# JuliaMeshless/WhatsThePoint.jl

Hardware: AMD Instinct MI355X
Metric: Mpoints/sec per repel iter (k=21 KNN+force) (higher is better)
Workload: dtype f32

## Files before the change

### include/wtp.h

```cpp
#ifndef WTP_H
#define WTP_H

#include <stdint.h>

#ifdef __cplusplus
extern "C" {
#endif

typedef struct wtp_ctx wtp_ctx;

typedef enum wtp_status {
    WTP_OK = 0,
    WTP_ERR_ARG = 1,
    WTP_ERR_OOM = 2,
    WTP_ERR_HIP = 3,
    WTP_ERR_STATE = 4,
    WTP_ERR_NO_DEVICE = 5
} wtp_status;

typedef enum wtp_dtype { WTP_F32 = 0, WTP_F64 = 1 } wtp_dtype;

typedef enum wtp_force_kind {
    WTP_FORCE_INVERSE_DISTANCE = 0,
    WTP_FORCE_SPACING_EQUILIBRIUM = 1,
// ... 165 lines not shown
                   int64_t n_owned, const wtp_spacing_desc* spacing, const wtp_force_desc* force, int k,
                   double alpha_lo, double alpha_max);
int wtp_block_step(wtp_ctx* ctx, wtp_step_stats* stats, wtp_block_info* info);
int wtp_block_run(wtp_ctx* ctx, int n_iters, double* conv_out, wtp_step_stats* last, wtp_block_info* info);
int wtp_block_run_until(wtp_ctx* ctx, int max_iters, double tol, int stall_after, double cv_target, double* conv_out,
                        int* n_done, int* reason, wtp_step_stats* last);
int wtp_block_get(wtp_ctx* ctx, void* d_xyz_out, int64_t* d_gid_out, int64_t cap, int64_t* n_owned);
int wtp_block_close(wtp_ctx* ctx);
int wtp_block_grid(int nranks, int p_out[3]);
int wtp_block_morton_rank(int ix, int iy, int iz, const int p[3]);
int wtp_comm_exchange_peers(wtp_ctx* ctx, int n_msgs, const int* peers, const void* const* d_send, const int64_t* n_send,
                            void* const* d_recv, const int64_t* n_recv);
int wtp_comm_allgather_dev(wtp_ctx* ctx, const void* d_send, void* d_recv, int64_t bytes);

int wtp_relax_set_coverage(wtp_ctx* ctx, int axis, double lo, double hi);
int wtp_relax_set_coverage_box(wtp_ctx* ctx, const double lo[3], const double hi[3]);

int wtp_relax_set_fixed_dev(wtp_ctx* ctx, const void* d_fixed4, int64_t n_fixed_new);


int wtp_timers_get(wtp_ctx* ctx, double out[4]);
int wtp_timers_reset(wtp_ctx* ctx);
int wtp_debug_diag(wtp_ctx* ctx, unsigned long long out[16]);

int wtp_gen_uniform_dev(wtp_ctx* ctx, uint64_t seed, int64_t first, int64_t n, int dim, int dtype,
                        void* d_out);

#ifdef __cplusplus
}
#endif
#endif
```

### whatsthepoint.jl_amd/_lib.py

```python
from __future__ import annotations

import ctypes as C
import os
import subprocess

_HERE = os.path.dirname(os.path.abspath(__file__))
CSRC = os.path.join(_HERE, "csrc")
SO_PATH = os.environ.get("WTP_LIB") or os.path.join(CSRC, "libwtp.so")

WTP_OK, WTP_ERR_ARG, WTP_ERR_OOM, WTP_ERR_HIP, WTP_ERR_STATE, WTP_ERR_NO_DEVICE = range(6)
WTP_F32, WTP_F64 = 0, 1
WTP_SPACING_CONSTANT, WTP_SPACING_PER_POINT, WTP_SPACING_LOGLIKE, WTP_SPACING_BOUNDARY_LAYER = range(4)


class WtpError(RuntimeError):

    def __init__(self, code, msg):
        super().__init__(f"libwtp status {code}: {msg}")
        self.code = code


class WtpArgumentError(ValueError):
    """WTP_ERR_ARG: the reference throws ArgumentError for the same input (src/repel.jl:74)."""

# ... 85 lines not shown
                                    C.POINTER(C.c_double), C.POINTER(C.c_double), C.POINTER(_vp), C.POINTER(_vp), _i64,
                                    C.POINTER(_i64)]),
    "wtp_relax_set_coverage": (_i, [_vp, _i, _d, _d]),
    "wtp_relax_set_coverage_box": (_i, [_vp, C.POINTER(C.c_double), C.POINTER(C.c_double)]),
    "wtp_comm_unique_id": (_i, [_vp, _vp]),
    "wtp_comm_init": (_i, [_vp, _vp, _i, _i]),
    "wtp_comm_finalize": (_i, [_vp]),
    "wtp_comm_exchange_rows": (_i, [_vp, _i, _i, _vp, _i64, _vp, _i64, _vp, _vp, _i64, C.POINTER(_i64), C.POINTER(_i64)]),
    "wtp_comm_allreduce_stats": (_i, [_vp, C.POINTER(StepStats)]),
    "wtp_block_set_transport": (_i, [_vp, C.POINTER(Transport)]),
    "wtp_block_open": (_i, [_vp, C.POINTER(BlockDesc), _vp, _vp, _i64, C.POINTER(SpacingDesc), C.POINTER(ForceDesc), _i, _d, _d]),
    "wtp_block_step": (_i, [_vp, C.POINTER(StepStats), C.POINTER(BlockInfo)]),
    "wtp_block_run": (_i, [_vp, _i, _vp, C.POINTER(StepStats), C.POINTER(BlockInfo)]),
    "wtp_block_run_until": (_i, [_vp, _i, _d, _i, _d, _vp, C.POINTER(_i), C.POINTER(_i), C.POINTER(StepStats)]),
    "wtp_block_get": (_i, [_vp, _vp, _vp, _i64, C.POINTER(_i64)]),
    "wtp_block_close": (_i, [_vp]),
    "wtp_block_grid": (_i, [_i, C.POINTER(_i)]),
    "wtp_block_morton_rank": (_i, [_i, _i, _i, C.POINTER(_i)]),
    "wtp_comm_exchange_peers": (_i, [_vp, _i, C.POINTER(_i), C.POINTER(_vp), C.POINTER(_i64), C.POINTER(_vp), C.POINTER(_i64)]),
    "wtp_comm_allgather_dev": (_i, [_vp, _vp, _vp, _i64]),
    "wtp_timers_get": (_i, [_vp, C.POINTER(_d)]),
    "wtp_timers_reset": (_i, [_vp]),
    "wtp_debug_diag": (_i, [_vp, C.POINTER(C.c_ulonglong)]),
    "wtp_gen_uniform_dev": (_i, [_vp, C.c_uint64, _i64, _i64, _i, _i, _vp]),
}

_lib = None


def build(verbose: bool = False) -> str:
    res = subprocess.run(["make", "-C", CSRC, "-j4"], capture_output=True, text=True)
    if res.returncode != 0:
        raise RuntimeError("building libwtp.so failed:\n" + res.stdout[-4000:] + res.stderr[-4000:])
    if verbose:
        print(res.stdout[-2000:])
    return SO_PATH


def load():
    global _lib
    if _lib is not None:
        return _lib
    if not os.path.exists(SO_PATH):
        raise ImportError(
            f"{SO_PATH} is missing: build it with `python -c 'import __graft_entry__ as g; g.build()'` "
            "(hipcc --offload-arch=gfx950).  There is no CPU fallback."
# ... 23 lines not shown
```

### whatsthepoint.jl_amd/csrc/wtp_api.hip

```cpp
#include <cmath>
#include <cstdlib>
#include <cstring>
#include <type_traits>

#include "wtp_internal.hpp"

namespace wtp {

static thread_local std::string g_create_err;

int fail(wtp_ctx* ctx, int code, const std::string& msg) {
    if (ctx)
        ctx->err = msg;
    else
        g_create_err = msg;
    return code;
}

int ensure(wtp_ctx* ctx, DevBuf& b, size_t bytes) {
    if (bytes == 0) bytes = 16;
    if (b.cap >= bytes) return WTP_OK;
    if (b.p) {
        hipFree(b.p);
        b.p = nullptr;
// ... 1070 lines not shown

static int relax_f64_ksel_sweep(wtp_ctx* ctx, SearchArgs<double>& a, int* sp) {
    RelaxState& r = ctx->relax;
    const int64_t n = r.n;
    const int kc = 24;
    int rc;
    if ((rc = ensure(ctx, ctx->f64k_s64, sizeof(double4) * (size_t)n))) return rc;
    if ((rc = ensure(ctx, ctx->f64k_slot, sizeof(int32_t) * (size_t)n))) return rc;
    if ((rc = ensure(ctx, ctx->f64k_lists, sizeof(int32_t) * 2 * (size_t)n))) return rc;
    if ((rc = ensure(ctx, ctx->f64k_cnt, 64))) return rc;
    const double4* snap = (const double4*)a.snap;
    SearchArgs<float> b{};
    b.fb_list = (int32_t*)ctx->f64k_lists.p;
    b.fb_count = (int32_t*)ctx->f64k_cnt.p;
    b.fb2_list = (int32_t*)ctx->f64k_lists.p + n;
    b.fb2_count = (int32_t*)ctx->f64k_cnt.p + 4;
    b.stop = ctx->stop_dev;
    b.diag = a.diag;
    *sp = span_begin(ctx, 0);
    WTP_HIP(ctx, hipMemsetAsync(ctx->f64k_cnt.p, 0, 64, ctx->stream));
    b.counters_cleared = 1;
    std::swap(ctx->grid, ctx->grid_b);
    std::swap(ctx->cell_start, ctx->cell_start_b);
    const void* ncells_session = ctx->ncells_dev;
    const bool box_session = ctx->box_active;
    const double* org4 = nullptr;
    rc = f64_candidates(ctx, snap, n, 3, kc, r.f64k_tune, b, *sp, &org4, [&](float4* sorted32) {
        return launch_relabel_slots(ctx, snap, sorted32, (double4*)ctx->f64k_s64.p, (int32_t*)ctx->f64k_slot.p, n);
    });
    std::swap(ctx->grid, ctx->grid_b);
    std::swap(ctx->cell_start, ctx->cell_start_b);
    ctx->ncells_dev = ncells_session;
    ctx->box_active = box_session;
    if (rc) return rc;
    return launch_refine_sweep_f64(ctx, a, (const double4*)ctx->f64k_s64.p, (const int32_t*)ctx->f64k_slot.p,
                                   (const int32_t*)ctx->cand_idx.p, (const float*)ctx->cand_dist.p, org4);
}

static bool grid_reusable(const wtp_ctx* ctx, int64_t n_fixed_next, bool head_swapped) {
    const RelaxState& r = ctx->relax;
    const bool head_ok = !head_swapped || (r.shard_grid_reuse && r.grid_fixed > 0 &&
                                           std::llabs((long long)(n_fixed_next - r.grid_fixed)) * 10 <= (long long)r.grid_fixed + 640);
    return r.grid_age < kGridReuseMax && !r.moved_by_hand && head_ok && !ctx->box_active;
}

static bool head_remeasures(const RelaxState& r, int64_t n_fixed_new) {
    const int64_t n_new = r.n - r.n_fixed + n_fixed_new;
    return r.cs2_bx > 0 && std::llabs((long long)(n_fixed_new - r.tuned_fixed)) * 20 > (long long)n_new;
}

template <typename T> static SweepRoute sweep_route(const wtp_ctx* ctx, const RelaxState& r) {
    if (ctx->force_generic) return SweepRoute::Exact;
    const bool clipped = r.force.kind == WTP_FORCE_CLIPPED_SPACING;
    if (clipped && r.k >= 2 && r.k < 32 && !ctx->full_select && !r.cs_disabled) {
// ... 132 lines not shown
            if (r.route == SweepRoute::Cs2) {
                Grid<float> hgf;
                memcpy(&hgf, &hg, sizeof(hgf));
                if ((rc = cs2_tune(ctx, r, hgf, rho_eff))) return rc;
            } else if (route_cs(r.route)) {
                int hc = (int)(HCELLS * rho_eff * 1.15) + 128;
                hc = (hc + 63) / 64 * 64;
                r.brick_hcap = hc < 640 ? 640 : (hc > 2560 ? 2560 : hc);
            }
            if (r.route == SweepRoute::Ksel) {
                if ((rc = ksel_tune<T>(ctx, r.tune, in, out, r.n, r.dim, r.k, hg, rho_eff))) return rc;
                g.rho = r.tune.rho;
            }
            r.tune.valid = true;
            r.tuned_fixed = r.n_fixed;
            r.grid_fixed = r.n_fixed;
            r.grid_age = 0;
        } else {
            const bool reuse = grid_reusable(ctx, r.n_fixed, ctx->hash_view.active);
            ctx->reuse_grid = reuse;
            r.grid_age = reuse ? r.grid_age + 1 : 0;
            if (!reuse) r.grid_fixed = r.n_fixed;
            ctx->topology_build = r.route == SweepRoute::F64Ksel;
            rc = build_hash<T>(ctx, in, out, r.n, r.dim, r.k, 0.0, g.rho, g.min_cell, r.tune.scale);
            ctx->topology_build = false;
            ctx->reuse_grid = false;
        }
        r.last_rho_cs = g.rho;
        span_end(ctx, sp);
        ctx->hash_view.active = false;
        if (rc) return rc;
        r.pending.active = false;
        r.bufS = t;
        r.bufP = t;
        r.have_tree = true;
        r.sweeps_since_rebuild = 0;
        r.moved_by_hand = false;
    }
    if (spacing_on_device(r.spacing_kind)) {
        int sps = span_begin(ctx, 2);
        rc = launch_spacing_session<T>(ctx, (const Pt<T>*)ctx->pts[r.bufP].p, r.n, r.n_fixed, ctx->kd_nodes.p, ctx->kd_m,
                                       r.spacing_kind, r.sp_p0, r.sp_p1, r.sp_p2, (T*)ctx->spacing_pp.p,
                                       (int32_t*)ctx->sp_hint.p - r.aux_off, r.have_tree ? (const int32_t*)ctx->cell_start.p : nullptr,
                                       ctx->grid.p, (Pt<T>*)ctx->sp_cert.p - r.aux_off);
        span_end(ctx, sps);
        if (rc) return rc;
    }
    const bool fresh = (r.bufS == r.bufP);
    const int o = pick_free(r, r.bufS, r.bufP);
    if ((rc = ensure(ctx, ctx->pts[o], sizeof(Pt<T>) * (size_t)(r.n + r.shard_extra)))) return rc;
// ... 31 lines not shown
        }
    }
    if ((rc = ensure(ctx, ctx->diag, 128))) return rc;
    a.diag = (unsigned long long*)ctx->diag.p;
    a.brick_hcap = route_cs(r.route) ? r.brick_hcap : (r.route == SweepRoute::Ksel ? r.tune.hcap : 0);
    a.cs2_bx = route_cs(r.route) ? r.cs2_bx : 0;
    a.cs2_chunked = (r.spacing_kind != WTP_SPACING_CONSTANT || r.cs2_rho > 1.6) ? 1 : 0;
    a.ksel_bx = r.route == SweepRoute::Ksel ? r.tune.bx : 0;
    if (r.route == SweepRoute::Ksel) a.cap_count = (float)ksel_cap_count(r.k);
    if (route == SweepRoute::Select || route == SweepRoute::Cs || route == SweepRoute::Cs2) {
        a.gamma_cap = (T)kGammaCapSweep;
        a.cap_count = (float)(4.18879 * kGammaCapSweep * kGammaCapSweep * kGammaCapSweep * ctx->rho * (a.k + 1) / 22.0);
    }
    if (route == SweepRoute::Cs64 || route == SweepRoute::Cs64Wave) a.gamma_cap = (T)kGammaCap;
    a.tnn_frac = (T)kTnnFrac;
    a.cover_axis = r.cover_axis;
    a.cover_lo = (T)r.cover_lo;
    a.cover_hi = (T)r.cover_hi;
    for (int ax = 0; ax < 3; ++ax) {
        a.cover_lo3[ax] = (T)r.cover_lo3[ax];
        a.cover_hi3[ax] = (T)r.cover_hi3[ax];
    }
    a.uncovered = (int32_t*)ctx->fb_count.p + 8;
    if (!ctx->counters_clean) WTP_HIP(ctx, hipMemsetAsync(ctx->fb_count.p, 0, 64, ctx->stream));
    ctx->counters_clean = false;
    a.used_brick = a.used_wave = a.used_generic = 0;
    if ((rc = launch_sweep<T>(ctx, a, route, ball && route_ball(route)))) return rc;
    int sp = span_begin(ctx, 2);
    if (r.wall_active) {
        char* wf = (char*)ctx->wall_flags.p;
        rc = launch_mesh_constrain<T>(ctx, a.query, a.out, r.n, r.n_fixed, r.wall_offset, (const uint8_t*)wf,
                                      (uint8_t*)wf + r.wall_nm, (int32_t*)ctx->wall_tri.p, (int32_t*)ctx->wall_hint.p,
                                      (int32_t*)ctx->fb_count.p + 12);
        if (rc) return rc;
    }
    rc = launch_reduce_partials(ctx, a.partials, a.n_partials, a.used_brick, a.used_wave, a.used_generic, a.fb_count,
                                a.uncovered, r.wall_active ? (const int32_t*)ctx->fb_count.p + 12 : nullptr, d_slot);
    span_end(ctx, sp);
    if (rc) return rc;
    r.bufOld = r.bufP;
    r.bufP = o;
    r.can_revert = true;
    r.have_point_data = true;
    r.sweeps_since_rebuild += 1;
    return WTP_OK;
}

static int relax_step_any(wtp_ctx* ctx, int rebuild, wtp_step_stats* d_slot) {
    return by_dtype(ctx->relax.dtype, [&](auto t) { return relax_step_t<decltype(t)>(ctx, rebuild, d_slot); });
}
int wtp::relax_step_enqueue(wtp_ctx* ctx, int rebuild, wtp_step_stats* d_slot) { return relax_step_any(ctx, rebuild, d_slot); }

int wtp::relax_prerank(wtp_ctx* ctx, int64_t n_fixed_new) {
    RelaxState& r = ctx->relax;
    ctx->prerank.valid = false;
    if (!r.active || !r.tune.valid || !r.have_tree || r.pending.active) return WTP_OK;
    if (!grid_reusable(ctx, n_fixed_new, true) || head_remeasures(r, n_fixed_new)) return WTP_OK;
    const int64_t n_new = r.n - r.n_fixed + n_fixed_new;
    if (ctx->pts[r.bufP].cap < pt_size(r.dtype) * (size_t)(r.n + n_fixed_new)) return WTP_OK;
    const int k = (int64_t)r.k_req < n_new ? r.k_req : (int)n_new;
    return by_dtype(r.dtype, [&](auto t) {
        return prerank_old_snapshot<decltype(t)>(ctx, pts_of<decltype(t)>(ctx, r.bufP), r.n, (int32_t)r.n_fixed, n_new,
                                                 r.n + n_fixed_new, k, r.last_rho_cs, r.tune.scale);
    });
// ... 698 lines not shown
}

WTP_API int wtp_timers_get(wtp_ctx* ctx, double out[4]) {
    if (!ctx || !out) return WTP_ERR_ARG;
    hipSetDevice(ctx->device);
    spans_collect(ctx);
    out[0] = ctx->t_hash;
    out[1] = ctx->t_sweep;
    out[2] = ctx->t_other;
    out[3] = (double)ctx->n_sweep_launches;
    return WTP_OK;
}

WTP_API int wtp_timers_reset(wtp_ctx* ctx) {
    if (!ctx) return WTP_ERR_ARG;
    hipSetDevice(ctx->device);
    spans_collect(ctx);
    ctx->t_hash = ctx->t_sweep = ctx->t_other = 0;
    ctx->n_sweep_launches = 0;
    if (!ctx->timing_forced) ctx->timing = true;
    return WTP_OK;
}

WTP_API int wtp_debug_diag(wtp_ctx* ctx, unsigned long long out[16]) {
    if (!ctx || !out) return WTP_ERR_ARG;
    WTP_HIP(ctx, hipSetDevice(ctx->device));
    int rc;
    if ((rc = ensure(ctx, ctx->diag, 128))) return rc;
    WTP_HIP(ctx, hipMemcpyAsync(out, ctx->diag.p, 128, hipMemcpyDeviceToHost, ctx->stream));
    WTP_HIP(ctx, hipMemsetAsync(ctx->diag.p, 0, 128, ctx->stream));
    if ((rc = sync(ctx))) return rc;
    if (ctx->debug_kd) {
        unsigned long long kd[2] = {0, 0};
        wtp::debug_kd_steps(kd);
        fprintf(stderr, "[wtp] kd walk: %llu node visits by %llu wave-walks (%.1f per walk)\n", kd[0], kd[1], kd[1] ? (double)kd[0] / (double)kd[1] : 0.0);
    }
    return WTP_OK;
}

WTP_API int wtp_gen_uniform_dev(wtp_ctx* ctx, uint64_t seed, int64_t first, int64_t n, int dim, int dtype, void* d_out) {
    if (!ctx || !d_out || n < 0) return WTP_ERR_ARG;
    WTP_HIP(ctx, hipSetDevice(ctx->device));
    int rc = dtype == WTP_F32 ? launch_gen_uniform<float>(ctx, seed, first, n, dim, (float*)d_out)
                              : launch_gen_uniform<double>(ctx, seed, first, n, dim, (double*)d_out);
    if (rc) return rc;
    return sync(ctx);
// ... 3 lines not shown
```

### whatsthepoint.jl_amd/csrc/wtp_cs2.hip

```cpp
#include "wtp_device.hpp"

namespace wtp {

#ifndef WTP_DIAG
#define WTP_DIAG 0
#endif
#define CS_STAMP(i)                                                 \
    if (WTP_DIAG) {                                                 \
        const unsigned long long t_ = __builtin_amdgcn_s_memtime(); \
        dt[i] += t_ - t_last;                                       \
        t_last = t_;                                                \
    }

constexpr int kCsThreads = 256;
constexpr int kCsSlab = 16;
constexpr int kCsMaxBX = 61;
constexpr int kCsMaxCells = (kCsMaxBX + 2) * kCsSlab;
constexpr int kCsMaskSteps = 12;
constexpr int kCsSU = 8;
constexpr int kCsPadBytes = 2 * kCsSU * 16;
constexpr int kCsMaxQ = 512;
constexpr int kCsMiss = 16;
constexpr int kCsRun = 2 * kCsSlab + 2 * 4 + 3;

// ... 34 lines not shown
    yo = yi + dy * sc;
    zo = zi + dz * sc;
    return Fn * s;
}

__device__ inline void cs_acc_point(CsAcc& c, float force, float nd, float s, int32_t id, int32_t nn) {
    c.max_force = force > c.max_force ? force : c.max_force;
    const float rs = __builtin_amdgcn_rcpf(s), q0 = nd * rs;
    const double u = (double)__builtin_fmaf(__builtin_fmaf(-s, q0, nd), rs, q0);
    c.sum_u += u;
    c.sum_u2 += u * u;
    c.n_move += 1;
    if (nd < c.argmin_r || (nd == c.argmin_r && id < c.argmin_i)) {
        c.argmin_r = nd;
        c.argmin_i = id;
        c.argmin_j = nn;
    }
}

struct ForceCoefCs {
    float A, beta;
};
__device__ inline ForceCoefCs force_coef_cs(float beta, float u0) { return ForceCoefCs{u0 * u0, beta}; }

static size_t cs2_smem_bytes(int hcap) {
    return (size_t)hcap * 16 + kCsPadBytes + sizeof(Cs2Smem);
}

template <bool CH>
__global__ __launch_bounds__(kCsThreads, 4) void cs2_kernel(SearchArgs<float> a, int hcap, int BX) {
    if (a.stop && *a.stop) return;
    extern __shared__ __attribute__((aligned(16))) unsigned char smem_raw[];
    float4* pts = reinterpret_cast<float4*>(smem_raw);
    Cs2Smem* sm = reinterpret_cast<Cs2Smem*>(smem_raw + (size_t)hcap * 16 + kCsPadBytes);
    const int tid = threadIdx.x, lane = tid & 63;
    const int wave = __builtin_amdgcn_readfirstlane(tid >> 6);

    const Grid<float> g = *a.grid;
    const int K = a.k;
    const int HX = BX + 2, ncell = HX * kCsSlab;
    const int nbx = (g.n[0] + BX - 1) / BX, nby = (g.n[1] + 1) / 2, nbz = (g.n[2] + 1) / 2;
    const int nbricks = nbx * nby * nbz;
    CsAcc acc;
    acc.max_force = 0.f;
    acc.argmin_r = Lim<float>::inf();
    acc.sum_u = acc.sum_u2 = 0.0;
// ... 175 lines not shown
        }
#pragma unroll
        for (int j = 0; j < 4; ++j) v[j] = vn[j];
        if (next < b_end) load_points(v, pv);
        __syncthreads();

        CS_STAMP(7)
        if (WTP_DIAG) dt[8] += 1;
#ifdef CS_ABL_NOQUERY
        const int Q = 0;
#else
        const int Q = sm->qpref[BX];
#endif
        if (overflow || Q > kCsMaxQ) {
            for (int r4 = 0; r4 < 4; ++r4) {
                const int gy = oy + 1 + (r4 & 1), gz = oz + 1 + (r4 >> 1);
                if (gy >= g.n[1] || gz >= g.n[2]) continue;
                const int gx0 = bx * BX, gx1 = (gx0 + BX - 1) < g.n[0] - 1 ? (gx0 + BX - 1) : g.n[0] - 1;
                const int base = (gz * g.n[1] + gy) * g.n[0];
                const int s = a.cell_start[base + gx0], e = a.cell_start[base + gx1 + 1];
                for (int i = s + tid; i < e; i += kCsThreads) {
                    const int pos = atomicAdd(a.fb_count, 1);
                    a.fb_list[pos] = i;
                }
            }
            continue;
        }
        __builtin_amdgcn_s_setprio(1);
        for (int qb = 0; qb < Q; qb += kCsThreads) {
            const int q = qb + tid;
            const bool active = q < Q;
            int hx = 1, cellp = 5, slot = 0, gslot = 0;
            if (active) {
                hx = sm->qslab[q];
                const int off = q - (int)sm->qpref[hx - 1];
                const int b = hx * kCsSlab;
                const int s5 = sm->ls[b + 5], s6 = sm->ls[b + 6], s7 = sm->ls[b + 7];
                const int s9 = sm->ls[b + 9], s10 = sm->ls[b + 10];
                const int n56 = s7 - s5;
                if (off < n56) {
                    slot = s5 + off;
                    cellp = slot < s6 ? 5 : 6;
                } else {
                    slot = s9 + (off - n56);
                    cellp = slot < s10 ? 9 : 10;
                }
                gslot = (int)sm->hglobal[b + cellp] + (slot - (int)sm->ls[b + cellp]);
            }
            if (!active) continue;
            const uint32_t qoff = (uint32_t)slot * 16u;
            const float4 qp = pts[slot];
            const int32_t qid = w_to_id(qp.w);
            if (qid < a.n_fixed) {
                a.out[gslot] = qp;
                a.forces[gslot] = 0.f;
                a.nn_dist[gslot] = Lim<float>::inf();
                a.nn_id[gslot] = -1;
                continue;
            }
            const int hy = cellp & 3, hz = cellp >> 2;
            const int cx = ox + hx, cy = oy + hy, cz = oz + hz;
            float s = s_c, inv_s2 = inv_s2_c, lim = lim_c;
            bool cs_fail = false;
            if (!const_ok) {
                if (a.spacing_pp) {
                    s = a.spacing_pp[qid];
                    inv_s2 = 1.f / (s * s);
                    lim = (a.u0 * a.u0) * (s * s);
                }
                cs_fail = !(lim <= safe_radius2(g, qp.x, qp.y, qp.z, cx, cy, cz, 1));
            }
            const int Pf = (hx - 1) * kCsSlab + (hz - 1) * 4 + (hy - 1);
            const uint32_t pa_first = (uint32_t)sm->ls[Pf] * 16u, ea_all = (uint32_t)sm->ls[Pf + kCsRun] * 16u;
            constexpr uint32_t kChunk = (uint32_t)(kCsMaskSteps * kCsSU) * 16u;
            bool giveup = (ea_all - pa_first) > (CH ? 4u : 1u) * kChunk;
            const uint32_t ea_all_s = giveup ? pa_first : ea_all;
            const float tau_s = (cs_fail || giveup) ? -1.f : lim * (1.f + 0x1p-21f);
// ... 135 lines not shown
                    asm("v_ffbh_u32 %0, %1" : "=v"(l) : "v"(cur));
                    off = cur != 0u ? (hi ? base1 : base0) + (l << 4) : qoff;
                    const uint32_t rest = cur & ~(0x80000000u >> (l & 31u));
                    m1 = hi ? rest : m1;
                    m0 = hi ? m0 : rest;
                };
                while (__any((m1 | m0) != 0u)) {
                    if (WTP_DIAG) dt[13] += 1;
                    uint32_t o1, o2;
                    take(o1);
                    take(o2);
                    const float4 c1 = lds_pt(smem_raw, o1), c2 = lds_pt(smem_raw, o2);
                    visit(c1);
                    visit(c2);
                }
            }
            if (!CH || !__any(pa_first + cbase + kChunk < ea_all_s)) break;
            }
            const int n_lim = n_oth + 1;
            CS_STAMP(3)
            if (cs_fail || giveup || n_lim > K || coincident) {
                const int pos = atomicAdd(a.fb_count, 1);
                a.fb_list[pos] = gslot;
                continue;
            }
            float4 o;
            const float f = cs_step_point(a, s, qp.x, qp.y, qp.z, Fx, Fy, Fz, o.x, o.y, o.z);
            o.w = qp.w;
            a.out[gslot] = o;
            a.forces[gslot] = f;
            const bool has = nid != 0x7FFFFFFF;
            if (has) {
                const float nd = wsqrt(nd2);
                if (reaches_past_cover<float>(a, qp.x, qp.y, qp.z, lim)) atomicAdd(a.uncovered, 1);
                a.nn_dist[gslot] = nd;
                a.nn_id[gslot] = nid;
                cs_acc_point(acc, f, nd, s, qid, nid);
            }
            const unsigned long long mm = __ballot(!has);
            if (mm) {
                const int base_m = sm->miss_n[wave];
                if (!has) {
                    const int pos = base_m + (int)__popcll(mm & ((1ull << lane) - 1ull));
                    if (pos < kCsMiss) {
                        CsMiss e;
                        e.pa = pa_first;
                        e.ea = ea_all;
                        e.qoff = qoff;
                        e.gslot = gslot;
                        e.qid = qid;
                        e.f = f;
                        e.s = s;
                        e.g2 = safe_radius2(g, qp.x, qp.y, qp.z, cx, cy, cz, 1);
                        sm->miss[wave][pos] = e;
                    } else {
                        const int p2 = atomicAdd(a.fb_count, 1);
                        a.fb_list[p2] = gslot;
                    }
                }
                const int first = __ffsll((long long)mm) - 1;
                const int tot = base_m + (int)__popcll(mm);
                __builtin_amdgcn_wave_barrier();
                if (lane == first) sm->miss_n[wave] = tot < kCsMiss ? tot : kCsMiss;
                __builtin_amdgcn_wave_barrier();
            }
            CS_STAMP(4)
        }

        {
            const int nm = __builtin_amdgcn_readfirstlane(sm->miss_n[wave]);
            for (int m = 0; m < nm; ++m) {
                const CsMiss e = sm->miss[wave][m];
                const float4 qp = lds_pt(smem_raw, e.qoff);
                float bd = Lim<float>::inf();
                int32_t bi = 0x7FFFFFFF;
                for (uint32_t p = e.pa + (uint32_t)lane * 16u; p < e.ea; p += 64u * 16u) {
                    const float4 c = lds_pt(smem_raw, p);
                    const int32_t cid = w_to_id(c.w);
                    const float d = dist2<float>(qp.x, qp.y, qp.z, c.x, c.y, c.z);
                    if (cid != e.qid && lex_lt(d, cid, bd, bi)) {
// ... 144 lines not shown
            }
        }
#pragma unroll
        for (int dlt = 8; dlt >= 1; dlt >>= 1) {
            const float od = __shfl_xor(bd, dlt, 64);
            const int32_t oi = __shfl_xor(bi, dlt, 64);
            if (lex_lt(od, oi, bd, bi)) {
                bd = od;
                bi = oi;
            }
        }
        if (l16 == 0 && on) {
            const float g2 = safe_radius2(g, qp.x, qp.y, qp.z, cx, cy, cz, 2);
            if (bi != 0x7FFFFFFF && bd <= g2) {
                const float s = a.spacing_pp ? a.spacing_pp[qid] : a.spacing_const;
                const float nd = wsqrt(bd);
                if (reaches_past_cover<float>(a, qp.x, qp.y, qp.z, bd)) atomicAdd(a.uncovered, 1);
                a.nn_dist[gslot] = nd;
                a.nn_id[gslot] = bi;
                acc_point<float>(acc, a.forces[gslot], nd, s, qid, bi);
            } else {
                const int pos = atomicAdd(a.fb_count, 1);
                a.fb_list[pos] = gslot;
            }
        }
    }
    acc_block_reduce(acc, sacc);
    if (threadIdx.x == 0) acc_store(&a.partials[part_base + blockIdx.x], acc);
}

constexpr int kBallThreads = 256;
constexpr int kBallBlocksMax = 3072;
constexpr int kBallRMax = 4;
#ifndef WTP_BALL_LANES
#define WTP_BALL_LANES 8
#endif
constexpr int kBallLanes = WTP_BALL_LANES;
constexpr int kBallPerWave = 64 / kBallLanes;
__global__ __launch_bounds__(kBallThreads, 6) void cs_ball_kernel(SearchArgs<float> a, const int32_t* __restrict__ list,
                                                               const int32_t* __restrict__ list_count,
                                                               int32_t* __restrict__ out_list, int32_t* __restrict__ out_count,
                                                               int part_base) {
    if (a.stop && *a.stop) return;
    __shared__ Acc sacc[kBallThreads / 64];
    const Grid<float> g = *a.grid;
    const int n = *list_count;
// ... 144 lines not shown
            const int gy = by * 2 + (r4 & 1), gz = bz * 2 + (r4 >> 1);
            rs[r4] = re[r4] = 0;
            if (gy >= g.n[1] || gz >= g.n[2]) continue;
            const int base = (gz * g.n[1] + gy) * g.n[0];
            rs[r4] = a.cell_start[base + gx0];
            re[r4] = a.cell_start[base + gx1 + 1];
        }
        for (int r4 = 0; r4 < 4 && is_dead; ++r4)
            for (int i = rs[r4]; i < re[r4] && is_dead; ++i) {
                const int32_t id = w_to_id(a.snap[i].w);
                if (id < a.n_fixed) {
                    is_dead = false;
                } else {
                    const float s = a.spacing_pp[id];
                    is_dead = (a.u0 * a.u0) * (s * s) > g2max;
                }
            }
        dead[brick] = is_dead ? 1 : 0;
        if (is_dead) {
            const int q = (re[0] - rs[0]) + (re[1] - rs[1]) + (re[2] - rs[2]) + (re[3] - rs[3]);
            if (q > 0) {
                int pos = atomicAdd(a.fb_count, q);
                for (int r4 = 0; r4 < 4; ++r4)
                    for (int i = rs[r4]; i < re[r4]; ++i) a.fb_list[pos++] = i;
            }
        }
    }
}

int launch_cs2_dead(wtp_ctx* ctx, SearchArgs<float>& a, uint8_t* d_dead, int dead_cap) {
    hipLaunchKernelGGL(cs2_dead_kernel, dim3(1024), dim3(256), 0, ctx->stream, a, a.cs2_bx, d_dead, dead_cap);
    WTP_HIP(ctx, hipGetLastError());
    return WTP_OK;
}

int launch_cs2(wtp_ctx* ctx, SearchArgs<float>& a) {
    const int hcap = a.brick_hcap, BX = a.cs2_bx;
    if (hcap < 64 || hcap > 4096 || BX < 1 || BX > kCsMaxBX)
        return fail(ctx, WTP_ERR_STATE, "compact-support sweep launched without a brick geometry");
    const size_t smem = cs2_smem_bytes(hcap);
    const bool chunked = a.cs2_chunked != 0;
    const void* fn = chunked ? (const void*)cs2_kernel<true> : (const void*)cs2_kernel<false>;
    if (ctx->cs2_smem != smem || ctx->cs2_fn != fn) {
        WTP_HIP(ctx, hipFuncSetAttribute(fn, hipFuncAttributeMaxDynamicSharedMemorySize, (int)smem));
        int occ = 0;
        hipError_t e = chunked ? hipOccupancyMaxActiveBlocksPerMultiprocessor(&occ, cs2_kernel<true>, kCsThreads, smem)
                               : hipOccupancyMaxActiveBlocksPerMultiprocessor(&occ, cs2_kernel<false>, kCsThreads, smem);
// ... 28 lines not shown
```

### whatsthepoint.jl_amd/csrc/wtp_hash.hip

```cpp
#include "wtp_device.hpp"

namespace wtp {

static constexpr int kThreads = 256;

template <typename T>
__global__ void load_points_kernel(const T* __restrict__ xyz, Pt<T>* __restrict__ out, int64_t n, int dim) {
    int64_t i = (int64_t)blockIdx.x * blockDim.x + threadIdx.x;
    int64_t stride = (int64_t)gridDim.x * blockDim.x;
    for (; i < n; i += stride) {
        Pt<T> p;
        p.x = xyz[i * dim + 0];
        p.y = xyz[i * dim + 1];
        p.z = dim == 3 ? xyz[i * dim + 2] : (T)0;
        p.w = id_to_w((T)0, (int32_t)i);
        out[i] = p;
    }
}

template <typename T>
__global__ void bbox_kernel(const Pt<T>* __restrict__ pts, int64_t n, T* __restrict__ part, int64_t v_old = 0,
                            int32_t v_fixed_old = 0) {
    __shared__ T sm[6][kThreads / 64];
    T mn[3] = {Lim<T>::inf(), Lim<T>::inf(), Lim<T>::inf()};
// ... 142 lines not shown
    for (int64_t base = (int64_t)blockIdx.x * blockDim.x; base < n; base += stride) {
        const int64_t i = base + threadIdx.x;
        bool valid = i < n;
        int cell = -1;
        if (valid) {
            Pt<T> p = pts[i];
            valid = !(i < v_old && w_to_id(p.w) < v_fixed_old);
            if (valid) {
                int cx = cell_coord(g, p.x, 0), cy = cell_coord(g, p.y, 1), cz = cell_coord(g, p.z, 2);
                cell = (cz * g.n[1] + cy) * g.n[0] + cx;
            }
        }
        const int prev = __shfl_up(cell, 1, 64);
        const bool head = (lane == 0) || (prev != cell);
        const unsigned long long heads = __ballot(head);
        const unsigned long long below = heads & ((2ull << lane) - 1ull);
        const int start = 63 - __builtin_clzll(below);
        const unsigned long long above = lane == 63 ? 0ull : (heads >> (lane + 1));
        const int len_to_end = above ? __builtin_ctzll(above) + 1 : 64 - lane;
        int r0 = 0;
        if (head && valid) {
            r0 = atomicAdd(&cell_cnt[cell], len_to_end);
            if (r0 != 0 && dirty) dirty[cell] = 1;
        }
        r0 = __shfl(r0, start, 64);
        if (valid) cell_rank[i] = r0 + (lane - start);
    }
}

static constexpr int kScanItems = 16;
static constexpr int kScanTile = kThreads * kScanItems;

__device__ inline int wave_incl_scan(int v) {
    int lane = threadIdx.x & 63;
#pragma unroll
    for (int d = 1; d < 64; d <<= 1) {
        int o = __shfl_up(v, d, 64);
        if (lane >= d) v += o;
    }
    return v;
}

__device__ inline int block_excl_scan(int v, int* total, int* sm ) {
    int incl = wave_incl_scan(v);
    int lane = threadIdx.x & 63, wave = threadIdx.x >> 6;
    if (lane == 63) sm[wave] = incl;
// ... 365 lines not shown
    const int64_t v_old = hv.active ? hv.n_old : 0;
    const int32_t v_fixed_old = hv.active ? hv.fixed_old : 0, v_shift = hv.active ? hv.id_shift : 0;
    const int nbb = grid_for(n_in, kThreads, 1024);
    int cap = 0, rc;
    bool fresh = false;
    if ((rc = hash_scratch(ctx, n, n_in, k, radius, rho_direct, cell_scale, &cap, &fresh))) return rc;
    const int nscan = (cap + kScanTile - 1) / kScanTile;

    Grid<T>* g = (Grid<T>*)ctx->grid.p;
    T* part = (T*)ctx->bbox_part.p;
    int32_t* cnt = (int32_t*)ctx->cell_cnt.p;
    int32_t* start = (int32_t*)ctx->cell_start.p;
    int32_t* cr = (int32_t*)ctx->cell_of.p;
    uint8_t* dirty = (uint8_t*)ctx->rank_of.p;
    int32_t* bs = (int32_t*)ctx->scan_tmp.p;
    hipStream_t st = ctx->stream;

    double rho_k = (dim == 3 ? 0.381 : 0.436) * (double)(k > 0 ? k : 21) * (ctx->rho / 8.0);
    if (rho_direct > 0) rho_k = rho_direct;
    if (rho_k < 1.0) rho_k = 1.0;

    const bool reuse = ctx->reuse_grid;
    ctx->reuse_grid = false;
    const Prerank pre = ctx->prerank;
    ctx->prerank.valid = false;
    const bool half_done = pre.valid && reuse && hv.active && !fresh && pre.in == (const void*)in && pre.n_old == v_old &&
                           pre.fixed_old == v_fixed_old && pre.cnt == (const void*)cnt && pre.cr == (const void*)cr &&
                           pre.dirty == (const void*)dirty;
    if (!half_done && (!ctx->hash_scratch_clean || fresh)) {
        WTP_HIP(ctx, hipMemsetAsync(cnt, 0, ctx->cell_cnt.cap, st));
        WTP_HIP(ctx, hipMemsetAsync(dirty, 0, ctx->rank_of.cap, st));
    }
    ctx->hash_scratch_clean = false;
    ctx->preranked_builds += half_done ? 1 : 0;
    if (!reuse) {
        hipLaunchKernelGGL(bbox_kernel<T>, dim3(nbb), dim3(kThreads), 0, st, in, n_in, part, v_old, v_fixed_old);
        hipLaunchKernelGGL(grid_setup_kernel<T>, dim3(1), dim3(64), 0, st, part, nbb, g, n, dim, rho_k, radius, min_cell,
                           cap, cell_scale, ctx->box_active ? (const double*)ctx->box_dev.p : (const double*)nullptr, ctx->stop_dev);
    }
    ctx->ncells_dev = &g->ncells;
    const int nb = grid_for(n_in, kThreads, 16384);
    if (half_done) {
        if (n_in > v_old)
            hipLaunchKernelGGL(cell_rank_kernel<T>, dim3(grid_for(n_in - v_old, kThreads, 16384)), dim3(kThreads), 0, st, in + v_old,
                               n_in - v_old, g, cnt, cr + v_old, ctx->topology_build ? (uint8_t*)nullptr : dirty, (int64_t)0, 0,
                               ctx->stop_dev);
    } else {
        hipLaunchKernelGGL(cell_rank_kernel<T>, dim3(nb), dim3(kThreads), 0, st, in, n_in, g, cnt, cr,
                           ctx->topology_build ? (uint8_t*)nullptr : dirty, v_old, v_fixed_old, ctx->stop_dev);
    }
    hipLaunchKernelGGL(scan_reduce_kernel<T>, dim3(nscan), dim3(kThreads), 0, st, cnt, g, bs);
    hipLaunchKernelGGL(scan_apply_kernel<T>, dim3(nscan), dim3(kThreads), 0, st, cnt, bs, g, start, ctx->stop_dev);
    hipLaunchKernelGGL(scatter_kernel<T>, dim3(nb), dim3(kThreads), 0, st, in, n_in, cr, g, start, out, v_old, v_fixed_old,
                       v_shift, ctx->stop_dev);
    if (!ctx->topology_build) {
        hipLaunchKernelGGL(canon_kernel<T>, dim3(grid_for((cap + 15) / 16, kThreads, 4096)), dim3(kThreads), 0, st, out, start,
                           dirty, g, ctx->stop_dev);
    }
    WTP_HIP(ctx, hipGetLastError());
    ctx->hash_scratch_clean = true;
    return WTP_OK;
}

template <typename T>
__global__ void unpermute_kernel(const Pt<T>* __restrict__ pts, int64_t n, int64_t n_fixed, int dim,
                                 T* __restrict__ out) {
    int64_t i = (int64_t)blockIdx.x * blockDim.x + threadIdx.x;
    int64_t stride = (int64_t)gridDim.x * blockDim.x;
    for (; i < n; i += stride) {
// ... 472 lines not shown
```

### whatsthepoint.jl_amd/csrc/wtp_internal.hpp

```cpp
#pragma once
#include <hip/hip_runtime.h>
#include <stdint.h>
#include <map>
#include <string>
#include <utility>
#include <vector>

#include "../../include/wtp.h"

namespace wtp {

template <typename T> struct PtOf;
template <> struct PtOf<float> { using type = float4; };
template <> struct PtOf<double> { using type = double4; };
template <typename T> using Pt = typename PtOf<T>::type;

template <typename F> inline auto by_dtype(int dtype, F&& f) { return dtype == WTP_F32 ? f(float{}) : f(double{}); }

__host__ __device__ inline float id_to_w(float, int32_t id) { return __builtin_bit_cast(float, id); }
__host__ __device__ inline double id_to_w(double, int32_t id) {
    return __builtin_bit_cast(double, (int64_t)id);
}
__host__ __device__ inline int32_t w_to_id(float w) { return __builtin_bit_cast(int32_t, w); }
__host__ __device__ inline int32_t w_to_id(double w) {
// ... 85 lines not shown
    int64_t rad_arena_cap;
    int32_t* rad_bricks;
    int32_t rad_dense;
    int32_t* fb_list;
    int32_t* fb_count;
    int32_t* fb2_list;
    int32_t* fb2_count;
    int32_t* nn_list;
    int32_t* nn_count;
    int32_t* ball_list;
    int32_t* ball_count;
    const int32_t* stop;
    int32_t cover_axis;
    T cover_lo, cover_hi;
    T cover_lo3[3], cover_hi3[3];
    int32_t* uncovered;
    T gamma_cap;
    float cap_count;
    T tnn_frac;
    int32_t brick_hcap;
    int32_t cs2_bx;
    const uint8_t* brick_dead;
    int32_t brick_dead_cap;
    int32_t cs2_chunked;
    int32_t counters_cleared;
    int32_t fb_r0;
    int32_t ksel_bx;
    unsigned long long* diag;
};

struct DevBuf {
    void* p = nullptr;
    size_t cap = 0;
    DevBuf() = default;
    DevBuf(const DevBuf&) = delete;
    DevBuf& operator=(const DevBuf&) = delete;
    DevBuf(DevBuf&& o) noexcept : p(o.p), cap(o.cap) {
        o.p = nullptr;
        o.cap = 0;
    }
    DevBuf& operator=(DevBuf&& o) noexcept {
        std::swap(p, o.p);
        std::swap(cap, o.cap);
        return *this;
    }
    ~DevBuf() {
// ... 49 lines not shown
    double spacing_const = 0, alpha_lo = 0, alpha_max = 0;
    ForceParams force{};
    int bufS = -1, bufP = -1, bufOld = -1;
    bool have_tree = false;
    bool can_revert = false;
    bool have_point_data = false;
    double spacing_max = 0;
    int brick_hcap = 0;
    GridTune tune;
    int grid_age = 0;
    int sweeps_since_rebuild = 0;
    bool moved_by_hand = false;
    double spacing_typ = 0;
    SweepRoute route = SweepRoute::Exact;
    bool cs_disabled = false;
    double cs2_rho = 0;
    int cs2_bx = 0;
    int64_t tuned_fixed = 0;
    double sp_p0 = 0, sp_p1 = 0, sp_p2 = 0;
    HashView pending;
    int64_t shard_extra = 0;
    int64_t aux_off = 0;
    int swap_target = -1;
    bool shard_grid_reuse = false;
    int64_t grid_fixed = -1;
    GridTune f64k_tune{true};
    double last_rho_cs = 0.0;
    bool wall_active = false;
    double wall_offset = 0;
    int64_t wall_nm = 0;
    int cover_axis = -1;
    double cover_lo = 0, cover_hi = 0;
    double cover_lo3[3] = {0, 0, 0}, cover_hi3[3] = {0, 0, 0};
};

}

struct wtp_ctx {
    int device = 0;
    hipStream_t stream = nullptr;
    hipStream_t own_stream = nullptr;
    std::string err;
    int sm_count = 256;
    double rho = 9.0;
    int force_generic = 0;
    int full_select = 0;
    int ksel = 1;
    int ball64 = 1;
    int f64_ksel = 1;
    int radius_dense = 1;
    int block_overlap = 1;
    bool debug = false;
    bool debug_kd = false;
    size_t cs2_smem = 0;
    const void* cs2_fn = nullptr;
    int cs2_occ = 0;
    std::map<std::pair<const void*, size_t>, int> launch_cache;
    wtp::GridTune knn_tune, knn64_tune;
    wtp::DevBuf pts[3];
    wtp::DevBuf raw_in;
    wtp::DevBuf cell_of, rank_of, cell_cnt, cell_start, scan_tmp;
    wtp::DevBuf grid, bbox_part, occ;
    wtp::HashView hash_view;
    wtp::DevBuf box_dev;
    bool topology_build = false;
    bool reuse_grid = false;
    bool box_active = false;
    const void* ncells_dev = nullptr;
    wtp::DevBuf idx_out, dist_out, counts_out;
    wtp::DevBuf cand_idx, cand_dist, f32_pts;
    wtp::DevBuf grid_b, cell_start_b, f64k_s64, f64k_slot, f64k_lists, f64k_cnt;
    wtp::DevBuf forces, nn_dist, nn_id, spacing_pp;
    wtp::DevBuf partials, stats, fb_list, fb_count, fb2_list, fb2_count, nn_list;
    wtp::DevBuf rad_pos;
    wtp::DevBuf rad_bricks;
    bool rad_dense_attr[2] = {false, false};
    bool rad_dense_used = false;
    wtp::DevBuf rad_tmp, rad_done;
    wtp::DevBuf rad_arena, rad_arena_off;
    wtp::DevBuf brick_dead;
    wtp::Prerank prerank;
    int64_t preranked_builds = 0;
    hipStream_t comm_stream = nullptr;
    hipEvent_t ev_comm_a = nullptr, ev_comm_b = nullptr;
    bool hash_scratch_clean = false;
    bool counters_clean = false;
    wtp::DevBuf stop_state;
    const int32_t* stop_dev = nullptr;
    wtp::DevBuf scratch;
// ... 197 lines not shown
```

Baseline: 12480.

## Carry per-point cell keys from sweep kernel into next hash rebuild

The Cs2 sweep kernel now writes each moved point's grid cell index into a side buffer, with -1 for fallback points. On the next grid-reusing hash rebuild, a new keyed rank kernel reads these keys instead of recomputing cell coordinates from positions. A grid generation counter and the buffer identity guard against stale keys. This adds an extra int32 store per point in the sweep in exchange for skipping a point load and the cell math in the rank pass. Debug APIs to toggle the keys and snapshot state are also added.

```diff
diff --git a/include/wtp.h b/include/wtp.h
--- a/include/wtp.h
+++ b/include/wtp.h
@@ -211,6 +211,8 @@
 int wtp_timers_get(wtp_ctx* ctx, double out[4]);
 int wtp_timers_reset(wtp_ctx* ctx);
 int wtp_debug_diag(wtp_ctx* ctx, unsigned long long out[16]);
+int wtp_debug_cell_keys(wtp_ctx* ctx, int enable, int64_t* keyed_builds);
+int wtp_debug_snapshot(wtp_ctx* ctx, void* pts_out, int32_t* cell_start_out, int64_t* ncells);
 
 int wtp_gen_uniform_dev(wtp_ctx* ctx, uint64_t seed, int64_t first, int64_t n, int dim, int dtype,
                         void* d_out);
diff --git a/whatsthepoint.jl_amd/_lib.py b/whatsthepoint.jl_amd/_lib.py
--- a/whatsthepoint.jl_amd/_lib.py
+++ b/whatsthepoint.jl_amd/_lib.py
@@ -131,6 +131,8 @@
     "wtp_timers_get": (_i, [_vp, C.POINTER(_d)]),
     "wtp_timers_reset": (_i, [_vp]),
     "wtp_debug_diag": (_i, [_vp, C.POINTER(C.c_ulonglong)]),
+    "wtp_debug_cell_keys": (_i, [_vp, _i, C.POINTER(_i64)]),
+    "wtp_debug_snapshot": (_i, [_vp, _vp, C.POINTER(C.c_int32), C.POINTER(_i64)]),
     "wtp_gen_uniform_dev": (_i, [_vp, C.c_uint64, _i64, _i64, _i, _i, _vp]),
 }
 
diff --git a/whatsthepoint.jl_amd/csrc/wtp_api.hip b/whatsthepoint.jl_amd/csrc/wtp_api.hip
--- a/whatsthepoint.jl_amd/csrc/wtp_api.hip
+++ b/whatsthepoint.jl_amd/csrc/wtp_api.hip
@@ -1116,6 +1116,7 @@
     b.counters_cleared = 1;
     std::swap(ctx->grid, ctx->grid_b);
     std::swap(ctx->cell_start, ctx->cell_start_b);
+    ctx->grid_gen += 1;
     const void* ncells_session = ctx->ncells_dev;
     const bool box_session = ctx->box_active;
     const double* org4 = nullptr;
@@ -1124,6 +1125,7 @@
     });
     std::swap(ctx->grid, ctx->grid_b);
     std::swap(ctx->cell_start, ctx->cell_start_b);
+    ctx->grid_gen += 1;
     ctx->ncells_dev = ncells_session;
     ctx->box_active = box_session;
     if (rc) return rc;
@@ -1302,10 +1304,14 @@
             r.grid_age = reuse ? r.grid_age + 1 : 0;
             if (!reuse) r.grid_fixed = r.n_fixed;
             ctx->topology_build = r.route == SweepRoute::F64Ksel;
+            if (reuse && r.keys_buf == r.bufP && r.keys_grid == ctx->grid_gen && ctx->cell_keys_on)
+                ctx->hash_keys = (const int32_t*)ctx->cell_key.p;
             rc = build_hash<T>(ctx, in, out, r.n, r.dim, r.k, 0.0, g.rho, g.min_cell, r.tune.scale);
             ctx->topology_build = false;
             ctx->reuse_grid = false;
+            ctx->hash_keys = nullptr;
         }
+        r.keys_buf = -1;
         r.last_rho_cs = g.rho;
         span_end(ctx, sp);
         ctx->hash_view.active = false;
@@ -1383,6 +1389,13 @@
         a.cover_hi3[ax] = (T)r.cover_hi3[ax];
     }
     a.uncovered = (int32_t*)ctx->fb_count.p + 8;
+    const bool keys = route == SweepRoute::Cs2 && !a.cs2_chunked && ctx->cell_keys_on && !r.wall_active &&
+                      !r.shard_grid_reuse && grid_reusable(ctx, r.n_fixed, false);
+    if (keys) {
+        if ((rc = ensure(ctx, ctx->cell_key, sizeof(int32_t) * (size_t)r.n))) return rc;
+        a.cell_key = (int32_t*)ctx->cell_key.p;
+    }
+    r.keys_buf = -1;
     if (!ctx->counters_clean) WTP_HIP(ctx, hipMemsetAsync(ctx->fb_count.p, 0, 64, ctx->stream));
     ctx->counters_clean = false;
     a.used_brick = a.used_wave = a.used_generic = 0;
@@ -1401,6 +1414,10 @@
     if (rc) return rc;
     r.bufOld = r.bufP;
     r.bufP = o;
+    if (keys) {
+        r.keys_buf = o;
+        r.keys_grid = ctx->grid_gen;
+    }
     r.can_revert = true;
     r.have_point_data = true;
     r.sweeps_since_rebuild += 1;
@@ -2145,6 +2162,31 @@
     return WTP_OK;
 }
 
+WTP_API int wtp_debug_cell_keys(wtp_ctx* ctx, int enable, int64_t* keyed_builds) {
+    if (!ctx) return WTP_ERR_ARG;
+    if (enable >= 0) ctx->cell_keys_on = enable != 0;
+    if (keyed_builds) *keyed_builds = ctx->keyed_builds;
+    return WTP_OK;
+}
+
+WTP_API int wtp_debug_snapshot(wtp_ctx* ctx, void* pts_out, int32_t* cell_start_out, int64_t* ncells_out) {
+    int rc = need_session(ctx, __func__);
+    if (rc) return rc;
+    const RelaxState& r = ctx->relax;
+    if (!r.have_tree || !ctx->ncells_dev) return fail(ctx, WTP_ERR_STATE, "wtp_debug_snapshot: no snapshot built yet");
+    WTP_HIP(ctx, hipSetDevice(ctx->device));
+    int32_t ncells = 0;
+    WTP_HIP(ctx, hipMemcpyAsync(&ncells, ctx->ncells_dev, sizeof(int32_t), hipMemcpyDeviceToHost, ctx->stream));
+    if ((rc = sync(ctx))) return rc;
+    if (ncells_out) *ncells_out = ncells;
+    if (pts_out)
+        WTP_HIP(ctx, hipMemcpyAsync(pts_out, ctx->pts[r.bufS].p, pt_size(r.dtype) * (size_t)r.n, hipMemcpyDeviceToHost, ctx->stream));
+    if (cell_start_out)
+        WTP_HIP(ctx, hipMemcpyAsync(cell_start_out, ctx->cell_start.p, sizeof(int32_t) * ((size_t)ncells + 1), hipMemcpyDeviceToHost,
+                                    ctx->stream));
+    return sync(ctx);
+}
+
 WTP_API int wtp_debug_diag(wtp_ctx* ctx, unsigned long long out[16]) {
     if (!ctx || !out) return WTP_ERR_ARG;
     WTP_HIP(ctx, hipSetDevice(ctx->device));
diff --git a/whatsthepoint.jl_amd/csrc/wtp_cs2.hip b/whatsthepoint.jl_amd/csrc/wtp_cs2.hip
--- a/whatsthepoint.jl_amd/csrc/wtp_cs2.hip
+++ b/whatsthepoint.jl_amd/csrc/wtp_cs2.hip
@@ -80,6 +80,11 @@
     float A, beta;
 };
 __device__ inline ForceCoefCs force_coef_cs(float beta, float u0) { return ForceCoefCs{u0 * u0, beta}; }
+
+__device__ inline int32_t cs_cell_key(const Grid<float>& g, const float4& p) {
+    const int cx = cell_coord(g, p.x, 0), cy = cell_coord(g, p.y, 1), cz = cell_coord(g, p.z, 2);
+    return (cz * g.n[1] + cy) * g.n[0] + cx;
+}
 
 static size_t cs2_smem_bytes(int hcap) {
     return (size_t)hcap * 16 + kCsPadBytes + sizeof(Cs2Smem);
@@ -301,6 +306,7 @@
                 for (int i = s + tid; i < e; i += kCsThreads) {
                     const int pos = atomicAdd(a.fb_count, 1);
                     a.fb_list[pos] = i;
+                    if (!CH && a.cell_key) a.cell_key[i] = -1;
                 }
             }
             continue;
@@ -332,6 +338,7 @@
             const int32_t qid = w_to_id(qp.w);
             if (qid < a.n_fixed) {
                 a.out[gslot] = qp;
+                if (!CH && a.cell_key) a.cell_key[gslot] = cs_cell_key(g, qp);
                 a.forces[gslot] = 0.f;
                 a.nn_dist[gslot] = Lim<float>::inf();
                 a.nn_id[gslot] = -1;
@@ -513,12 +520,14 @@
             if (cs_fail || giveup || n_lim > K || coincident) {
                 const int pos = atomicAdd(a.fb_count, 1);
                 a.fb_list[pos] = gslot;
+                if (!CH && a.cell_key) a.cell_key[gslot] = -1;
                 continue;
             }
             float4 o;
             const float f = cs_step_point(a, s, qp.x, qp.y, qp.z, Fx, Fy, Fz, o.x, o.y, o.z);
             o.w = qp.w;
             a.out[gslot] = o;
+            if (!CH && a.cell_key) a.cell_key[gslot] = cs_cell_key(g, o);
             a.forces[gslot] = f;
             const bool has = nid != 0x7FFFFFFF;
             if (has) {
@@ -547,6 +556,7 @@
                     } else {
                         const int p2 = atomicAdd(a.fb_count, 1);
                         a.fb_list[p2] = gslot;
+                        if (!CH && a.cell_key) a.cell_key[gslot] = -1;
                     }
                 }
                 const int first = __ffsll((long long)mm) - 1;
@@ -737,6 +747,7 @@
             } else {
                 const int pos = atomicAdd(a.fb_count, 1);
                 a.fb_list[pos] = gslot;
+                if (a.cell_key) a.cell_key[gslot] = -1;
             }
         }
     }
@@ -927,7 +938,10 @@
             if (q > 0) {
                 int pos = atomicAdd(a.fb_count, q);
                 for (int r4 = 0; r4 < 4; ++r4)
-                    for (int i = rs[r4]; i < re[r4]; ++i) a.fb_list[pos++] = i;
+                    for (int i = rs[r4]; i < re[r4]; ++i) {
+                        a.fb_list[pos++] = i;
+                        if (a.cell_key) a.cell_key[i] = -1;
+                    }
             }
         }
     }
diff --git a/whatsthepoint.jl_amd/csrc/wtp_hash.hip b/whatsthepoint.jl_amd/csrc/wtp_hash.hip
--- a/whatsthepoint.jl_amd/csrc/wtp_hash.hip
+++ b/whatsthepoint.jl_amd/csrc/wtp_hash.hip
@@ -188,6 +188,44 @@
         if (head && valid) {
             r0 = atomicAdd(&cell_cnt[cell], len_to_end);
             if (r0 != 0 && dirty) dirty[cell] = 1;
+        }
+        r0 = __shfl(r0, start, 64);
+        if (valid) cell_rank[i] = r0 + (lane - start);
+    }
+}
+
+template <typename T>
+__global__ void cell_rank_key_kernel(const Pt<T>* __restrict__ pts, const int32_t* __restrict__ keys, int64_t n,
+                                     const Grid<T>* __restrict__ gp, int32_t* __restrict__ cell_cnt,
+                                     int32_t* __restrict__ cell_rank, uint8_t* __restrict__ dirty,
+                                     const int32_t* __restrict__ stop) {
+    if (stop && *stop) return;
+    const int lane = threadIdx.x & 63;
+    const int64_t stride = (int64_t)gridDim.x * blockDim.x;
+    for (int64_t base = (int64_t)blockIdx.x * blockDim.x; base < n; base += stride) {
+        const int64_t i = base + threadIdx.x;
+        const bool valid = i < n;
+        int cell = -1;
+        if (valid) {
+            cell = keys[i];
+            if (cell < 0) {
+                const Grid<T> g = *gp;
+                const Pt<T> p = pts[i];
+                const int cx = cell_coord(g, p.x, 0), cy = cell_coord(g, p.y, 1), cz = cell_coord(g, p.z, 2);
+                cell = (cz * g.n[1] + cy) * g.n[0] + cx;
+            }
+        }
+        const int prev = __shfl_up(cell, 1, 64);
+        const bool head = (lane == 0) || (prev != cell);
+        const unsigned long long heads = __ballot(head);
+        const unsigned long long below = heads & ((2ull << lane) - 1ull);
+        const int start = 63 - __builtin_clzll(below);
+        const unsigned long long above = lane == 63 ? 0ull : (heads >> (lane + 1));
+        const int len_to_end = above ? __builtin_ctzll(above) + 1 : 64 - lane;
+        int r0 = 0;
+        if (head && valid) {
+            r0 = atomicAdd(&cell_cnt[cell], len_to_end);
+            if (r0 != 0) dirty[cell] = 1;
         }
         r0 = __shfl(r0, start, 64);
         if (valid) cell_rank[i] = r0 + (lane - start);
@@ -599,6 +637,8 @@
 
     const bool reuse = ctx->reuse_grid;
     ctx->reuse_grid = false;
+    const int32_t* keys = ctx->hash_keys;
+    ctx->hash_keys = nullptr;
     const Prerank pre = ctx->prerank;
     ctx->prerank.valid = false;
     const bool half_done = pre.valid && reuse && hv.active && !fresh && pre.in == (const void*)in && pre.n_old == v_old &&
@@ -610,6 +650,10 @@
     }
     ctx->hash_scratch_clean = false;
     ctx->preranked_builds += half_done ? 1 : 0;
+    const bool keyed = keys && reuse && !hv.active && !half_done && !ctx->topology_build &&
+                       ctx->cell_key.p == (const void*)keys && ctx->cell_key.cap >= sizeof(int32_t) * (size_t)n_in;
+    ctx->keyed_builds += keyed ? 1 : 0;
+    if (!reuse) ctx->grid_gen += 1;
     if (!reuse) {
         hipLaunchKernelGGL(bbox_kernel<T>, dim3(nbb), dim3(kThreads), 0, st, in, n_in, part, v_old, v_fixed_old);
         hipLaunchKernelGGL(grid_setup_kernel<T>, dim3(1), dim3(64), 0, st, part, nbb, g, n, dim, rho_k, radius, min_cell,
@@ -622,6 +666,9 @@
             hipLaunchKernelGGL(cell_rank_kernel<T>, dim3(grid_for(n_in - v_old, kThreads, 16384)), dim3(kThreads), 0, st, in + v_old,
                                n_in - v_old, g, cnt, cr + v_old, ctx->topology_build ? (uint8_t*)nullptr : dirty, (int64_t)0, 0,
                                ctx->stop_dev);
+    } else if (keyed) {
+        hipLaunchKernelGGL(cell_rank_key_kernel<T>, dim3(nb), dim3(kThreads), 0, st, in, keys, n_in, g, cnt, cr, dirty,
+                           ctx->stop_dev);
     } else {
         hipLaunchKernelGGL(cell_rank_kernel<T>, dim3(nb), dim3(kThreads), 0, st, in, n_in, g, cnt, cr,
                            ctx->topology_build ? (uint8_t*)nullptr : dirty, v_old, v_fixed_old, ctx->stop_dev);
diff --git a/whatsthepoint.jl_amd/csrc/wtp_internal.hpp b/whatsthepoint.jl_amd/csrc/wtp_internal.hpp
--- a/whatsthepoint.jl_amd/csrc/wtp_internal.hpp
+++ b/whatsthepoint.jl_amd/csrc/wtp_internal.hpp
@@ -131,6 +131,7 @@
     int32_t cs2_bx;
     const uint8_t* brick_dead;
     int32_t brick_dead_cap;
+    int32_t* cell_key;
     int32_t cs2_chunked;
     int32_t counters_cleared;
     int32_t fb_r0;
@@ -226,6 +227,8 @@
     int64_t shard_extra = 0;
     int64_t aux_off = 0;
     int swap_target = -1;
+    int keys_buf = -1;
+    uint64_t keys_grid = 0;
     bool shard_grid_reuse = false;
     int64_t grid_fixed = -1;
     GridTune f64k_tune{true};
@@ -269,6 +272,11 @@
     wtp::DevBuf box_dev;
     bool topology_build = false;
     bool reuse_grid = false;
+    const int32_t* hash_keys = nullptr;
+    uint64_t grid_gen = 0;
+    bool cell_keys_on = true;
+    int64_t keyed_builds = 0;
+    wtp::DevBuf cell_key;
     bool box_active = false;
     const void* ncells_dev = nullptr;
     wtp::DevBuf idx_out, dist_out, counts_out;
```

Result: no change. 12490 (median of 6 runs) (+0.1%).
